# jinli99/iShapEditing

Hardware: AMD Instinct MI355X
Metric: end-to-end drag-edit wall-clock (s) per shape (lower is better)
Workload: dtype f16; 1 GPU; C3 chair drag-edit: 3 handle->target pairs, 40 guided iterations (UNet fwd + drag gradient + UNet input-grad bwd + DDPM update) + 256^3 occupancy decode; unet=421M params, 1x96x128x128 latent, fp16 torso, r1=12, scale=1200

## Files before the change

### ishapediting_amd/csrc/misc.hip

```cpp
#include "misc.h"

__global__ __launch_bounds__(256) void nchw_to_nhwc_kernel(const float* __restrict__ src, half_t* __restrict__ dst,
                                                           int C, int HW, int Cpad, int ytiles, uint4* __restrict__ zero, long long zero_n16) {
  __shared__ float tile[32][33];
  const int n = blockIdx.z;
  if ((int)blockIdx.y >= ytiles) {
    const long long nb = (long long)gridDim.x * (gridDim.y - ytiles) * gridDim.z;
    const long long b = blockIdx.x + (long long)gridDim.x * ((blockIdx.y - ytiles) + (long long)(gridDim.y - ytiles) * blockIdx.z);
    for (long long i = b * 256 + threadIdx.x; i < zero_n16; i += nb * 256) zero[i] = make_uint4(0u, 0u, 0u, 0u);
    return;
  }
  const int p0 = blockIdx.x * 32, c0 = blockIdx.y * 32;
  const int tx = threadIdx.x & 31, ty = threadIdx.x >> 5;
  for (int j = ty; j < 32; j += 8) {
    int c = c0 + j, p = p0 + tx;
    tile[j][tx] = (c < C && p < HW) ? src[((long long)n * C + c) * HW + p] : 0.f;
  }
  __syncthreads();
  for (int j = ty; j < 32; j += 8) {
    int p = p0 + j, c = c0 + tx;
    if (p < HW && c < Cpad) dst[((long long)n * HW + p) * Cpad + c] = (half_t)tile[tx][j];
  }
}
int nchw_f32_to_nhwc_f16(const float* src, half_t* dst, int N, int C, int HW, int Cpad, hipStream_t s, void* zero, size_t zero_bytes) {
// ... 43 lines not shown
  const int tx = threadIdx.x & 31, ty = threadIdx.x >> 5;
  for (int j = ty; j < 32; j += 8) {
    int c = c0 + j, p = p0 + tx;
    tile[j][tx] = (c < C && p < HW) ? (float)src[((long long)n * C + c) * HW + p] * mul : 0.f;
  }
  __syncthreads();
  for (int j = ty; j < 32; j += 8) {
    int p = p0 + j, c = c0 + tx;
    if (p < HW && c < ld) dst[((long long)n * HW + p) * ld + c] = (half_t)tile[tx][j];
  }
}
int nchw_to_nhwc_f16_scaled(const void* src, int src_f32, half_t* dst, int N, int C, int HW, int ld, float mul,
                            hipStream_t s) {
  dim3 g(ceil_div(HW, 32), ceil_div(ld, 32), N);
  if (src_f32) hipLaunchKernelGGL(nchw_any_to_nhwc_kernel<float>, g, dim3(256), 0, s, (const float*)src, dst, C, HW, ld, mul);
  else hipLaunchKernelGGL(nchw_any_to_nhwc_kernel<half_t>, g, dim3(256), 0, s, (const half_t*)src, dst, C, HW, ld, mul);
  ISHAP_CHECK_HIP(hipGetLastError());
  return 0;
}

__global__ void concat2_kernel(const half_t* __restrict__ a, const half_t* __restrict__ b, half_t* __restrict__ o,
                               long long M, int Ca, int Cb, const long long* __restrict__ sa,
                               const long long* __restrict__ sb, long long* __restrict__ so, int N) {
  if (so && blockIdx.x == 0) {
    const int Cc = Ca + Cb;
    for (int i = threadIdx.x; i < N * Cc * 2; i += blockDim.x) {
      const int k = i & 1, c = (i >> 1) % Cc, n = (i >> 1) / Cc;
      so[i] = c < Ca ? sa[(n * Ca + c) * 2 + k] : sb[(n * Cb + (c - Ca)) * 2 + k];
    }
  }
  const int CV = (Ca + Cb) >> 3, CVa = Ca >> 3;
  const long long total = M * CV;
  for (long long i = (long long)blockIdx.x * blockDim.x + threadIdx.x; i < total; i += (long long)gridDim.x * blockDim.x) {
    long long m = i / CV;
    int cv = (int)(i % CV);
    half8 v = cv < CVa ? *reinterpret_cast<const half8*>(a + m * Ca + cv * 8)
                       : *reinterpret_cast<const half8*>(b + m * Cb + (cv - CVa) * 8);
    *reinterpret_cast<half8*>(o + m * (Ca + Cb) + cv * 8) = v;
  }
}
int concat2(const half_t* a, const half_t* b, half_t* o, long long M, int Ca, int Cb, hipStream_t s, const long long* sa,
            const long long* sb, long long* so, int N) {
  long long total = M * ((Ca + Cb) / 8);
  int blocks = (int)std::min<long long>((total + 255) / 256, 4096);
  hipLaunchKernelGGL(concat2_kernel, dim3(blocks), dim3(256), 0, s, a, b, o, M, Ca, Cb, sa, sb, so, N);
  ISHAP_CHECK_HIP(hipGetLastError());
  return 0;
}

__global__ void add_kernel(const half_t* __restrict__ a, const half_t* __restrict__ b, half_t* __restrict__ o, long long nvec) {
  for (long long i = (long long)blockIdx.x * blockDim.x + threadIdx.x; i < nvec; i += (long long)gridDim.x * blockDim.x) {
    half8 x = reinterpret_cast<const half8*>(a)[i], y = reinterpret_cast<const half8*>(b)[i], r;
#pragma unroll
    for (int k = 0; k < 8; ++k) r[k] = (half_t)((float)x[k] + (float)y[k]);
    reinterpret_cast<half8*>(o)[i] = r;
  }
}
int add_f16(const half_t* a, const half_t* b, half_t* o, long long n, hipStream_t s) {
  long long nvec = n / 8;
  int blocks = (int)std::min<long long>((nvec + 255) / 256, 4096);
  hipLaunchKernelGGL(add_kernel, dim3(blocks), dim3(256), 0, s, a, b, o, nvec);
  ISHAP_CHECK_HIP(hipGetLastError());
  return 0;
}


__global__ void timestep_embedding_kernel(TsArg t, float* __restrict__ out, int dim) {
  const int n = blockIdx.x;
  const int half = dim / 2;
  for (int j = threadIdx.x; j < half; j += blockDim.x) {
    float f = expf(-logf(10000.f) * (float)j / (float)half);
    float a = t.t[n] * f;
    out[n * dim + j] = cosf(a);
    out[n * dim + half + j] = sinf(a);
  }
  if ((dim & 1) && threadIdx.x == 0) out[n * dim + dim - 1] = 0.f;
}
int timestep_embedding(const TsArg& t, float* out, int N, int dim, hipStream_t s) {
  hipLaunchKernelGGL(timestep_embedding_kernel, dim3(N), dim3(128), 0, s, t, out, dim);
  ISHAP_CHECK_HIP(hipGetLastError());
  return 0;
}

__global__ __launch_bounds__(256) void gemv_kernel(const float* __restrict__ W, const float* __restrict__ b,
                                                   const float* __restrict__ in, float* __restrict__ out, int rows, int K,
                                                   int N, int silu_in) {
  const int row = blockIdx.x * 4 + (threadIdx.x >> 6);
  const int lane = threadIdx.x & 63;
  if (row >= rows) return;
  const float* w = W + (long long)row * K;
  for (int n = 0; n < N; ++n) {
    float acc = 0.f;
    for (int k = lane * 4; k < K; k += 256) {
      f32x4 wv = *reinterpret_cast<const f32x4*>(w + k);
      f32x4 xv = *reinterpret_cast<const f32x4*>(in + (long long)n * K + k);
#pragma unroll
      for (int i = 0; i < 4; ++i) {
        float x = xv[i];
        if (silu_in) x = x / (1.f + __expf(-x));
        acc += wv[i] * x;
      }
    }
    for (int o = 32; o > 0; o >>= 1) acc += __shfl_xor(acc, o);
    if (lane == 0) out[(long long)n * rows + row] = acc + b[row];
  }
}
int gemv_f32(const float* W, const float* b, const float* in, float* out, int rows, int K, int N, int silu_in,
             hipStream_t s) {
  ISHAP_REQUIRE(K % 4 == 0, "gemv K % 4");
  hipLaunchKernelGGL(gemv_kernel, dim3(ceil_div(rows, 4)), dim3(256), 0, s, W, b, in, out, rows, K, N, silu_in);
  ISHAP_CHECK_HIP(hipGetLastError());
  return 0;
}

__global__ void pack_conv_kernel(const float* __restrict__ w, half_t* __restrict__ dst, int O, int I, int taps,
                                 int rows_pad, int cpad, int transpose_flip, int dst_ld, int col_off) {
  const long long total = (long long)rows_pad * taps * cpad;
  for (long long i = (long long)blockIdx.x * blockDim.x + threadIdx.x; i < total; i += (long long)gridDim.x * blockDim.x) {
    int c = (int)(i % cpad);
    int tap = (int)((i / cpad) % taps);
    int r = (int)(i / ((long long)cpad * taps));
    float v = 0.f;
    if (!transpose_flip) {
      if (r < O && c < I) v = w[((long long)r * I + c) * taps + tap];
    } else {
      if (r < I && c < O) v = w[((long long)c * I + r) * taps + (taps - 1 - tap)];
    }
    dst[(long long)r * dst_ld + col_off + tap * cpad + c] = (half_t)v;
  }
}
int pack_conv_weight(const float* w, half_t* dst, int O, int I, int taps, int rows_pad, int cpad, int transpose_flip,
                     hipStream_t s, int dst_ld, int col_off) {
  long long total = (long long)rows_pad * taps * cpad;
  int blocks = (int)std::min<long long>((total + 255) / 256, 8192);
  hipLaunchKernelGGL(pack_conv_kernel, dim3(blocks), dim3(256), 0, s, w, dst, O, I, taps, rows_pad, cpad, transpose_flip,
                     dst_ld ? dst_ld : taps * cpad, col_off);
  ISHAP_CHECK_HIP(hipGetLastError());
  return 0;
}

__global__ void pack_conv_split_kernel(const float* __restrict__ w, half_t* __restrict__ dst, int O, int I, int taps,
                                       int rows_pad) {
  const int cpad = 3 * I;
  const long long total = (long long)rows_pad * taps * cpad;
  for (long long i = (long long)blockIdx.x * blockDim.x + threadIdx.x; i < total; i += (long long)gridDim.x * blockDim.x) {
    int c3 = (int)(i % cpad);
    int tap = (int)((i / cpad) % taps);
    int r = (int)(i / ((long long)cpad * taps));
    int part = c3 / I, c = c3 % I;
    float v = 0.f;
    if (r < O) {
      float f = w[((long long)r * I + c) * taps + tap];
      half_t hi = (half_t)f;
      v = (part < 2) ? (float)hi : (f - (float)hi);
    }
    dst[i] = (half_t)v;
  }
}
int pack_conv_weight_split(const float* w, half_t* dst, int O, int I, int taps, int rows_pad, hipStream_t s) {
  long long total = (long long)rows_pad * taps * 3 * I;
  int blocks = (int)std::min<long long>((total + 255) / 256, 8192);
  hipLaunchKernelGGL(pack_conv_split_kernel, dim3(blocks), dim3(256), 0, s, w, dst, O, I, taps, rows_pad);
  ISHAP_CHECK_HIP(hipGetLastError());
  return 0;
}

__global__ void round_f16_kernel(const float* __restrict__ src, float* __restrict__ dst, long long n) {
  for (long long i = (long long)blockIdx.x * blockDim.x + threadIdx.x; i < n; i += (long long)gridDim.x * blockDim.x)
    dst[i] = (float)(half_t)src[i];
}
int round_through_f16(const float* src, float* dst, long long n, hipStream_t s) {
  int blocks = (int)std::min<long long>((n + 255) / 256, 4096);
  hipLaunchKernelGGL(round_f16_kernel, dim3(blocks), dim3(256), 0, s, src, dst, n);
  ISHAP_CHECK_HIP(hipGetLastError());
  return 0;
}

__global__ __launch_bounds__(256) void nhwc_to_nchw_scaled_kernel(const half_t* __restrict__ src, float* __restrict__ dst,
                                                                  int C, int HW, int ld, const float* __restrict__ mul_dev) {
  __shared__ float tile[32][33];
  const float mul = mul_dev ? *mul_dev : 1.f;
  const int n = blockIdx.z;
  const int p0 = blockIdx.x * 32, c0 = blockIdx.y * 32;
  const int tx = threadIdx.x & 31, ty = threadIdx.x >> 5;
  for (int j = ty; j < 32; j += 8) {
    int p = p0 + j, c = c0 + tx;
    tile[j][tx] = (c < C && p < HW) ? (float)src[((long long)n * HW + p) * ld + c] * mul : 0.f;
  }
  __syncthreads();
  for (int j = ty; j < 32; j += 8) {
    int c = c0 + j, p = p0 + tx;
    if (c < C && p < HW) dst[((long long)n * C + c) * HW + p] = tile[tx][j];
  }
}
// ... 8 lines not shown
```

### ishapediting_amd/csrc/unet.hip

```cpp
#include "unet.h"

#include <cstring>

#include "attention.h"
#include "decode.h"
#include "misc.h"
#include "norm.h"

static int round_up(int a, int b) { return (a + b - 1) / b * b; }

static void init_conv(ConvW& c, const std::string& path, int cin, int cout, int taps) {
  c.path = path; c.cin = cin; c.cout = cout; c.taps = taps;
  c.kpad = round_up(cin, 32);
  c.cout_pad = round_up(cout, 32);
}

int unet_build(ishap_unet* u) {
  const ishap_unet_config& cfg = u->cfg;
  const int mc = cfg.model_channels;
  u->ted = mc * 4;
  u->in_pad = cfg.in_channels >= 64 ? round_up(cfg.in_channels, 64) : round_up(cfg.in_channels, 32);
  auto has_att = [&](int ds) {
    for (int i = 0; i < cfg.n_att; ++i) if (cfg.attention_ds[i] == ds) return true;
    return false;
  };
  auto heads_of = [&](int ch) { return ch / cfg.num_head_channels; };
  u->res.reserve(256);
  u->attn.reserve(64);
  int film = 0;
  auto add_res = [&](const std::string& path, int cin, int cout, bool up, bool down) {
    ResL r;
    r.path = path; r.cin = cin; r.cout = cout; r.up = up; r.down = down;
    r.n1.C = cin; r.n2.C = cout;
    init_conv(r.c1, path + ".in_layers.2", cin, cout, 9);
    init_conv(r.c2, path + ".out_layers.3", cout, cout, 9);
    r.has_skip = cin != cout;
    if (r.has_skip) init_conv(r.skip, path + ".skip_connection", cin, cout, 1);
    r.emb_off = film;
    film += 2 * cout;
    u->res.push_back(r);
    return (int)u->res.size() - 1;
  };
  auto add_attn = [&](const std::string& path, int ch) {
    AttnL a;
    a.path = path; a.C = ch; a.heads = heads_of(ch);
    a.n.C = ch;
    init_conv(a.qkv, path + ".qkv", ch, 3 * ch, 1);
    init_conv(a.proj, path + ".proj_out", ch, ch, 1);
    u->attn.push_back(a);
    return (int)u->attn.size() - 1;
  };

  int ch = cfg.channel_mult[0] * mc;
  int res = cfg.image_size;
  init_conv(u->stem, "input_blocks.0.0", cfg.in_channels, ch, 9);
  u->stem.kpad = u->in_pad;
  {
    BlockL b;
    b.name = "input_blocks.0";
    b.layers.push_back({0, 0});
    b.cin = cfg.in_channels; b.cout = ch; b.res_in = b.res_out = res;
    u->in_blocks.push_back(b);
  }
  std::vector<int> chans{ch};
  int ds = 1;
  for (int level = 0; level < cfg.n_mult; ++level) {
    for (int k = 0; k < cfg.num_res_blocks; ++k) {
      BlockL b;
      b.name = "input_blocks." + std::to_string(u->in_blocks.size());
      int cout = cfg.channel_mult[level] * mc;
      b.layers.push_back({1, add_res(b.name + ".0", ch, cout, false, false)});
      b.cin = ch; ch = cout; b.cout = ch; b.res_in = b.res_out = res;
      if (has_att(ds)) b.layers.push_back({2, add_attn(b.name + ".1", ch)});
      u->in_blocks.push_back(b);
      chans.push_back(ch);
    }
    if (level != cfg.n_mult - 1) {
      BlockL b;
      b.name = "input_blocks." + std::to_string(u->in_blocks.size());
      b.layers.push_back({1, add_res(b.name + ".0", ch, ch, false, true)});
      b.cin = b.cout = ch; b.res_in = res; b.res_out = res / 2;
      u->in_blocks.push_back(b);
      chans.push_back(ch);
      ds *= 2;
// ... 600 lines not shown
  u->marks_on = ishap_switch("ISHAP_BWD_MARKS", 0) != 0;
  u->device = device;
  int r = unet_build(u);
  if (r) { delete u; return r; }
  u->arena.dry = true;
  std::vector<float> ts(cfg->max_batch, 0.f);
  for (int nb = 1; nb <= cfg->max_batch && !r; ++nb) {
    r = unet_forward_impl(u, nullptr, ts.data(), nb, (int)u->out_blocks.size() - 1, nullptr, nullptr, 1, 0, true);
    if (!r) r = unet_backward_impl(u, nullptr, (const void*)0x1000, 0, nullptr, nullptr, 0, true);
  }
  if (r) { delete u; return r; }
  u->arena.dry = false;
  u->arena.cap = align_up(u->arena.high + (1 << 20), 1 << 20);
  ISHAP_CHECK_HIP(hipMalloc((void**)&u->arena.base, u->arena.cap));
  if (u->ws_floats) ISHAP_CHECK_HIP(hipMalloc((void**)&u->ws, u->ws_floats * sizeof(float)));
  ISHAP_CHECK_HIP(hipMalloc((void**)&u->gn_partial, std::max<size_t>(u->gn_partial_floats, 64) * sizeof(float)));
  u->stat_cap = (u->stat_high + 1023) / 1024 * 1024;
  ISHAP_CHECK_HIP(hipMalloc((void**)&u->stat_base, std::max<size_t>(u->stat_cap, 1024) * sizeof(long long)));
  if (u->attn_D_floats) ISHAP_CHECK_HIP(hipMalloc((void**)&u->attn_D, u->attn_D_floats * sizeof(float)));
  u->have_saved = false;
  *out = u;
  return 0;
}

void ishap_unet_destroy(ishap_unet* u) {
  if (!u) return;
  auto fr = [](void* p) { if (p) (void)hipFree(p); };
  auto frc = [&](ConvW& c) { fr(c.w); fr(c.wT); fr(c.bias); if (c.cat && c.cat_off == 0) fr(c.cat); };
  frc(u->stem); frc(u->head);
  fr(u->head_norm.gamma); fr(u->head_norm.beta);
  for (auto& r : u->res) {
    frc(r.c1); frc(r.c2); if (r.has_skip) frc(r.skip);
    fr(r.n1.gamma); fr(r.n1.beta); fr(r.n2.gamma); fr(r.n2.beta);
  }
  for (auto& a : u->attn) { frc(a.qkv); frc(a.proj); fr(a.n.gamma); fr(a.n.beta); }
  fr(u->te_w0); fr(u->te_b0); fr(u->te_w2); fr(u->te_b2); fr(u->emb_w); fr(u->emb_b);
  fr(u->d_temb); fr(u->d_e1); fr(u->d_emb); fr(u->d_film);
  fr(u->film_cache); fr(u->pc_temb); fr(u->pc_e1); fr(u->pc_emb);
  fr(u->ws_side); fr(u->gn_partial_side);
  fr(u->snap.arena); fr(u->snap.stat); fr(u->snap.film);
  if (u->side) (void)hipStreamDestroy(u->side);
  if (u->ev_fork) (void)hipEventDestroy(u->ev_fork);
  if (u->ev_tail) (void)hipEventDestroy(u->ev_tail);
  if (u->ev_mid) (void)hipEventDestroy(u->ev_mid);
  for (hipEvent_t ev : u->marks) (void)hipEventDestroy(ev);
  if (u->mark_tail_begin) (void)hipEventDestroy(u->mark_tail_begin);
  if (u->mark_tail_end) (void)hipEventDestroy(u->mark_tail_end);
  fr(u->arena.base); fr(u->ws); fr(u->gn_partial); fr(u->attn_D); fr(u->stat_base);
  delete u;
}

int ishap_unet_num_params(const ishap_unet* u) { return u ? (int)u->params.size() : 0; }

int ishap_unet_param_info(const ishap_unet* u, int index, char* name, int name_cap, int* ndim, long long* shape) {
  ISHAP_REQUIRE(u && index >= 0 && index < (int)u->params.size(), "param index");
  const ParamSlot& p = u->params[index];
  if (name && name_cap > 0) {
    std::strncpy(name, p.name.c_str(), name_cap - 1);
    name[name_cap - 1] = 0;
  }
  if (ndim) *ndim = p.ndim;
  if (shape) for (int i = 0; i < 4; ++i) shape[i] = p.shape[i];
  return 0;
}

int ishap_unet_load_param(ishap_unet* u, const char* name, const float* data, long long numel, void* stream) {
  ISHAP_REQUIRE(u && name && data, "null argument");
  auto it = u->param_index.find(name);
  ISHAP_REQUIRE(it != u->param_index.end(), std::string("unexpected key in state_dict: ") + name);
  ParamSlot& p = u->params[it->second];
  ISHAP_REQUIRE(p.numel() == numel, std::string("size mismatch for ") + name);
  ISHAP_CHECK_HIP(hipSetDevice(u->device));
  ISHAP_TRY(load_param(u, p, data, (hipStream_t)stream));
  if (!p.loaded) { p.loaded = true; u->n_loaded++; }
  u->film_cache_ts.clear();
  u->snap.valid = false;
  return 0;
}

int ishap_unet_prepare_timesteps(ishap_unet* u, const float* ts, int n, void* stream) {
  ISHAP_REQUIRE(u && (ts || n == 0) && n >= 0 && n <= 4096, "prepare_timesteps arguments");
  ISHAP_CHECK_HIP(hipSetDevice(u->device));
  hipStream_t s = (hipStream_t)stream;
  u->film_cache_ts.clear();
  if (u->film_cur != u->d_film) { u->have_saved = false; u->film_cur = u->d_film; u->film_cur_ld = u->film_rows; }
  if (n == 0) return 0;
  ISHAP_REQUIRE(u->n_loaded == (int)u->params.size(), "prepare_timesteps before all parameters are loaded");
  const int mc = u->cfg.model_channels;
  if ((size_t)n > u->film_cache_rows) {
    if (u->film_cache) ISHAP_CHECK_HIP(hipFree(u->film_cache));
    u->film_cache = nullptr;
    u->film_cache_rows = 0;
    ISHAP_CHECK_HIP(hipMalloc((void**)&u->film_cache, (size_t)n * u->film_rows * sizeof(float)));
    u->film_cache_rows = (size_t)n;
  }
  if (!u->pc_temb) {
    ISHAP_CHECK_HIP(hipMalloc((void**)&u->pc_temb, (size_t)16 * mc * sizeof(float)));
    ISHAP_CHECK_HIP(hipMalloc((void**)&u->pc_e1, (size_t)16 * u->ted * sizeof(float)));
    ISHAP_CHECK_HIP(hipMalloc((void**)&u->pc_emb, (size_t)16 * u->ted * sizeof(float)));
  }
  for (int c0 = 0; c0 < n; c0 += 16) {
    const int m = std::min(16, n - c0);
    TsArg ta;
    for (int i = 0; i < 16; ++i) ta.t[i] = i < m ? ts[c0 + i] : 0.f;
    ISHAP_TRY(timestep_embedding(ta, u->pc_temb, m, mc, s));
    ISHAP_TRY(gemv_f32(u->te_w0, u->te_b0, u->pc_temb, u->pc_e1, u->ted, mc, m, 0, s));
    ISHAP_TRY(gemv_f32(u->te_w2, u->te_b2, u->pc_e1, u->pc_emb, u->ted, u->ted, m, 1, s));
    ISHAP_TRY(gemv_f32(u->emb_w, u->emb_b, u->pc_emb, u->film_cache + (size_t)c0 * u->film_rows, u->film_rows, u->ted, m, 1, s));
  }
  u->film_cache_ts.assign(ts, ts + n);
  return 0;
}

int ishap_unet_params_loaded(const ishap_unet* u) { return u ? u->n_loaded : 0; }

int ishap_unet_join_tail(ishap_unet* u, void* stream) {
  ISHAP_REQUIRE(u, "null argument");
  ISHAP_CHECK_HIP(hipSetDevice(u->device));
  return unet_join_tail(u, (hipStream_t)stream);
}

int ishap_unet_run_tail(ishap_unet* u) {
  ISHAP_REQUIRE(u, "null argument");
  ISHAP_CHECK_HIP(hipSetDevice(u->device));
  return unet_run_tail(u);
}

int ishap_unet_forward(ishap_unet* u, const float* x, const float* timesteps, int N, int feat_layer, float* out,
                       void* inter_feat, int keep_for_backward, void* stream) {
  ISHAP_REQUIRE(u && x && timesteps && out, "null argument");
  ISHAP_REQUIRE(u->n_loaded == (int)u->params.size(), "missing keys: not every state_dict tensor has been loaded");
  ISHAP_TRY(ishap_check_status());
  ISHAP_CHECK_HIP(hipSetDevice(u->device));
  return unet_forward_impl(u, x, timesteps, N, feat_layer, out, inter_feat, keep_for_backward, (hipStream_t)stream, false);
}

int ishap_unet_tap_shape(const ishap_unet* u, int feat_layer, int* channels, int* size) {
  ISHAP_REQUIRE(u && feat_layer >= 0 && feat_layer < (int)u->out_blocks.size(), "feat_layer out of range");
  if (channels) *channels = u->out_blocks[feat_layer].cout;
  if (size) *size = u->out_blocks[feat_layer].res_out;
  return 0;
}

const void* ishap_unet_tap_ptr(const ishap_unet* u) { return u ? u->tap.p : nullptr; }

long long ishap_unet_workspace_bytes(const ishap_unet* u) {
  if (!u) return 0;
  return (long long)(u->arena.cap + u->ws_floats * sizeof(float) + u->gn_partial_floats * sizeof(float) +
                     u->stat_cap * sizeof(long long) + u->attn_D_floats * sizeof(float) + u->snap.bytes());
}

int ishap_unet_block_output(const ishap_unet* u, int group, int index, int* channels, int* size, void* dst_nchw_f16,
                            void* stream) {
  ISHAP_REQUIRE(u && group >= 0 && group <= 2, "group: 0 input_blocks, 1 middle_block, 2 output_blocks");
  const BlockL* b = nullptr;
  if (group == 0) { ISHAP_REQUIRE(index >= 0 && index < (int)u->in_blocks.size(), "input block index"); b = &u->in_blocks[index]; }
  else if (group == 1) b = &u->mid;
  else { ISHAP_REQUIRE(index >= 0 && index < (int)u->out_blocks.size(), "output block index"); b = &u->out_blocks[index]; }
  if (channels) *channels = b->cout;
  if (size) *size = b->res_out;
  if (!dst_nchw_f16) return 0;
  ISHAP_REQUIRE(u->have_saved && b->out.p, "block outputs stay resident only after a forward with keep_for_backward=1");
  ISHAP_REQUIRE(!(u->restored_partial && group == 2 && index > u->last_feat), "the restored snapshot holds the network up to the tap only");
  ISHAP_TRY(ishap_check_status());
  ISHAP_CHECK_HIP(hipSetDevice(u->device));
  ISHAP_TRY(unet_join_tail(const_cast<ishap_unet*>(u), (hipStream_t)stream));
// ... 125 lines not shown
```

### ishapediting_amd/drag_utils.py

```python
from __future__ import annotations

import argparse
import collections
import copy
import ctypes as C
import os
from argparse import Namespace
from typing import List, Optional

import numpy as np
import torch as th

from . import _lib
from .script_util import args_to_dict, create_model_and_diffusion, model_and_diffusion_defaults
from .triplane_decoder import MultiTriplane, decode_planes_grid, decode_volume, prepare_planes
from . import mesh as mesh_backend
from .volume import clean_volume


def get_args(argv=None):
    parser = argparse.ArgumentParser(description="Generate a set of triplane and their corresponding meshes")
    parser.add_argument("--resolution", type=str, default=128, required=False)
    parser.add_argument("--num_steps", type=int, default=200, required=False)
    parser.add_argument("--shape_resolution", type=int, default=256, required=False)
# ... 319 lines not shown
        if t.dtype != th.float16 or tuple(t.shape[-2:]) != (self.W * self.W, self.ld):
            raise ValueError(f"taps are fp16 [..., {self.W * self.W}, {self.ld}], got {t.dtype} {tuple(t.shape)}")
        t = t.to(self.device).contiguous()
        if t.dim() == 2:
            t = t[None]
        if t.dim() != 3 or t.shape[0] not in lead:
            raise ValueError(f"tap batch of {tuple(t.shape)} for {self.E} edits")
        return t

    def track_batch(self, edit_taps, orig_taps, sources, offsets=None, want_volume=False) -> List[Track]:
        self.setup(sources)
        edit, orig = self._tap(edit_taps, (self.E,)), self._tap(orig_taps, (1, self.E))
        H = self.handles
        if offsets is None:
            K_in = th.zeros((H, 3), dtype=th.int32, device=self.device)
        else:
            K_in = th.cat([th.as_tensor(np.asarray(o.detach().cpu() if th.is_tensor(o) else o)).to(th.int32).reshape(-1, 3)
                           for o in offsets]).to(self.device).contiguous()
            if K_in.shape[0] != H:
                raise ValueError(f"{K_in.shape[0]} offsets for {H} handles")
        K_out = th.empty_like(K_in)
        dist, dist0 = th.empty(H, dtype=th.float32, device=self.device), th.empty(H, dtype=th.float32, device=self.device)
        vol = th.empty((H, self.side ** 3), dtype=th.float32, device=self.device) if want_volume else None
        self.run_ptr(edit.data_ptr(), orig.data_ptr(), 0 if orig.shape[0] == 1 else orig[0].numel(), K_in, K_out, dist, dist0, vol)
        pos = self.positions(K_out)
        cut = lambda t, e: None if t is None else t[self.offsets[e]:self.offsets[e + 1]]
        return [Track(cut(K_out, e), cut(pos, e), cut(dist, e), cut(dist0, e), cut(vol, e)) for e in range(self.E)]

    def track(self, edit_tap, orig_tap, sources, offsets=None, want_volume=False) -> Track:
        return self.track_batch(edit_tap, orig_tap, [sources], None if offsets is None else [offsets], want_volume)[0]


class _LoopTrack:

    def __init__(self, tracker: HandleTracker, sources, steps_total: int, every: int):
        self.tracker, self.every = tracker.setup(sources), every
        rows = (steps_total + every - 1) // every
        H, dev = tracker.handles, tracker.device
        self.table = th.zeros((rows + 1, H, 3), dtype=th.int32, device=dev)
        self.dist = th.zeros((rows, H), dtype=th.float32, device=dev)
        self.dist0 = th.zeros((rows, H), dtype=th.float32, device=dev)
        self.steps: List[int] = []
        self._ptrs = (self.table.data_ptr(), self.dist.data_ptr(), self.dist0.data_ptr(), H)

    def step(self, n: int, edit_ptr: int, orig_ptr: int, orig_stride: int):
        if n % self.every:
            return
        r = len(self.steps)
        table, dist, dist0, H = self._ptrs
        self.tracker.run_raw(edit_ptr, orig_ptr, orig_stride, table + 12 * H * r, table + 12 * H * (r + 1), dist + 4 * H * r,
                             dist0 + 4 * H * r)
        self.steps.append(n)

    def results(self) -> List[dict]:
        t, r = self.tracker, len(self.steps)
        offs = self.table[1:r + 1].clone()
        pos = t.positions(offs)
        out = []
        for e in range(t.E):
            a, b = t.offsets[e], t.offsets[e + 1]
            out.append({"steps": list(self.steps), "offsets": offs[:, a:b], "positions": pos[:, a:b],
                        "dist": self.dist[:r, a:b].clone(), "dist0": self.dist0[:r, a:b].clone(), "radius": t.R, "patch": t.rp})
        return out


def synthesize_latent(model, diffusion, args=None, t1=None, t2=0, inter_latent_idx=None, inter_feat_idx=None, img=None,
                      calc_grad=False, **kwargs):
    if args is None:
        args = get_args()
    shape = (args.batch_size, 96, args.image_size, args.image_size)
    if img is None:
        img = th.randn(shape, device=next(model.parameters()).device)
        if calc_grad:
            img.requires_grad_(True)
    assert img.shape == shape
    if t1 is None:
        t1 = args.num_steps
    elif t1 == 0:
        return {"img": img[:args.num_samples], "inter_latent": [], "inter_feat": [], "pred_xstart": [], "model_output": None}
    sample_fun = diffusion.ddim_sample if getattr(args, "use_ddim", False) else diffusion.p_sample_guidance
    if calc_grad and getattr(args, "use_ddim", False):
        raise NotImplementedError("synthesize_latent(calc_grad=True) with use_ddim: the DDIM sampler has no autograd bridge")
    inter_latent, inter_feat, predict_x0, model_output, variance, noise = [], [], [], None, [], []
    with (th.enable_grad() if calc_grad else th.no_grad()):
        for i in range(t1 - 1, t2 - 1, -1):
            out = sample_fun(model, img, i, **kwargs)
            img = out["sample"]
            if inter_feat_idx is not None and i in inter_feat_idx:
                inter_feat.append(out["inter_feat"])
                if calc_grad:
                    noise.append(out["noise"].cpu())
                    variance.append(out["variance"].cpu())
            if inter_latent_idx is not None and i in inter_latent_idx:
                inter_latent.append(img)
                predict_x0.append(out["pred_xstart"])
            model_output = out["model_output"]
    return {"img": img[:args.num_samples], "inter_latent": inter_latent, "inter_feat": inter_feat,
            "pred_xstart": predict_x0, "model_output": model_output, "variance": variance, "noise": noise}


def load_triplane_stats(stats=None, stats_dir=None):
    if stats is not None:
        means, stds = stats
    else:
        files = [os.path.join(stats_dir, f) for f in ("means.npy", "stds.npy")] if stats_dir else []
        if not files or not all(os.path.exists(f) for f in files):
            raise FileNotFoundError(
                "train_triplane_opt needs the triplane statistics: pass stats=(means, stds) or set args.stats_dir to a "
                f"directory holding means.npy and stds.npy (stats_dir={stats_dir!r})")
        means, stds = (np.load(f) for f in files)
    means, stds = (np.asarray(v, dtype=np.float32).reshape(-1) for v in (means, stds))
    if means.size != 96 or stds.size != 96:
        raise ValueError(f"triplane statistics must hold 96 values each, not {means.size} and {stds.size}")
    return means, stds


class DragStuff:

    args = get_args()
    overlap_tail = None
    _w = None
    _shape_gen = 0
    _first_step = None

    @property
    def w(self):
        return self._w

    @w.setter
    def w(self, value):
        self._w = value
        self._shape_changed()

    def _shape_changed(self):
        self._shape_gen = self._shape_gen + 1
        self._first_step = None

    def _first_step_key(self, overlap):
        w = self._w
        return (self._shape_gen, id(self.model), id(w), getattr(w, "_version", None), tuple(w.shape), self.args.feat_layer,
                self.args.w_time, tuple(getattr(self.diffusion, "timestep_map", ())), bool(overlap))

    def __init__(self, device=None, args=None, max_edits=1):
        if args is not None:
            self.args = args
        if int(max_edits) < 1:
            raise ValueError(f"max_edits must be >= 1, not {max_edits}")
        self.max_edits = int(max_edits)
        self.device = th.device("cuda", th.cuda.current_device()) if device is None else th.device(device)
        self.model, self.diffusion = create_model_and_diffusion(
            **args_to_dict(self.args, model_and_diffusion_defaults().keys()), device=self.device, max_batch=self.max_edits)
        self.model.eval()
        self.decoder = MultiTriplane(1, input_dim=3, output_dim=1, device=self.device)
        self.decoder.eval()
        self.range = 1.
        self.middle = 0.
        self.latent_code = None
        self.w0 = None
        self.w = None
        self.r1 = 12
        self.offset1 = make_offsets(self.r1, self.device)
        self.voxel_size = 2. / self.args.shape_resolution
        self.train_flag = True
        self.targets = None
        self.sources = None
        self.mesh = None
        self.mesh0 = None
        self.volume = None
        self.clean = None
        self.refine = None
        self.noise = []
        self.variance = []
        self.variance_noise = []
        self.feature_guidance: List[th.Tensor] = []
        self.last_losses: List[float] = []
        self.last_track = None
        self._dk: Optional[DragKernels] = None
        self.step_noise = None
        self.w_batch = None
        self.w0_batch = None
        self.feature_guidance_batch: List[th.Tensor] = []
        self.meshes0 = []
        self.meshes = []
        self.volumes = []

    def set_offset1(self, r1):
        self.r1 = int(r1)
        self.offset1 = make_offsets(r1, self.device)

    def update_model_params(self, main_path):
        for files in os.listdir(main_path):
            if files.startswith("ddpm"):
                ddpm_path = os.path.join(main_path, files)
                for sub_file in os.listdir(ddpm_path):
                    if sub_file.startswith("ema"):
                        self.args.model_path = os.path.join(ddpm_path, sub_file)
                        break
            elif files.endswith(".pt"):
                self.args.decoder_ckpt = os.path.join(main_path, files)
        stat_path = os.path.join(main_path, "statistics")
        self.args.stats_dir = os.path.join(stat_path, os.listdir(stat_path)[0])
        self.args.save_dir = os.path.join("samples", main_path[9:] + "_samples")
        os.makedirs(self.args.save_dir, exist_ok=True)
        self.load_weights(th.load(self.args.model_path, map_location="cpu"),
                          th.load(self.args.decoder_ckpt, map_location="cpu"),
                          np.load(f"{self.args.stats_dir}/lower_bound.npy") if self.args.explicit_normalization else None,
                          np.load(f"{self.args.stats_dir}/upper_bound.npy") if self.args.explicit_normalization else None)

    def load_weights(self, unet_sd, decoder_sd, lower_bound=None, upper_bound=None):
        self._shape_changed()
        self.model.load_state_dict(unet_sd, strict=True)
        if self.args.use_fp16:
            self.model.convert_to_fp16()
        self.model.eval()
        if lower_bound is not None:
            mn = np.asarray(lower_bound).astype(np.float32).reshape(1, -1, 1, 1)
            mx = np.asarray(upper_bound).astype(np.float32).reshape(1, -1, 1, 1)
            self.range = (th.tensor(mx - mn) / 2).to(self.device)
            self.middle = th.tensor((mn + mx) / 2).to(self.device)
        else:
            self.range, self.middle = 1., 0.
        self.decoder.net.load_state_dict(decoder_sd)
        self.decoder.eval()

    def _noise(self, i, like):
        return None if self.step_noise is None else self.step_noise(i).to(like.device)

    def _denoise(self, img, t, each=None, **kwargs):
        for i in range(t - 1, -1, -1):
            img = self.diffusion.p_sample_guidance(self.model, img, i, feat_layer=self.args.feat_layer,
                                                   clip_denoised=self.args.clip_denoised, want_inter_feat=False,
                                                   noise=self._noise(i, img), want_noise=False, **kwargs)["sample"]
            if each is not None:
                each(i, img)
        return img

    def update_latent_params(self, img=None, **kwargs):
        if img is not None:
            if th.is_tensor(img):
                img = img.type(th.float32).to(self.device)
            elif type(img) is np.ndarray:
                img = th.tensor(img, dtype=th.float32, device=self.device)
            else:
                raise NotImplementedError("Unknown data type!")
        else:
            img = th.randn((1, 96, self.args.image_size, self.args.image_size), dtype=th.float32, device=self.device)
        self.latent_code = img.clone().detach()
        self._shape_changed()
        self.w_batch, self.w0_batch, self.feature_guidance_batch = None, None, []

        def record(i, img):
            if i == self.args.w_time:
                self.w = img.clone().detach()
                self.w0 = self.w.clone().detach()
            if i < self.args.w_time:
                self.feature_guidance.append(self.model.copy_tap(self.args.feat_layer)[0])

        img = self._denoise(img, self.args.num_steps, each=record, **kwargs)
        assert len(self.feature_guidance) == self.args.w_time
        self.mesh0 = self.get_mesh(tri_feat=img)
        self.mesh = copy.deepcopy(self.mesh0)
        return img

    def get_mesh(self, tri_feat=None, img=None, t=0):
        if tri_feat is None:
            img = img if img is not None else th.randn((1, 96, self.args.image_size, self.args.image_size)).to(self.device)
            tri_feat = self._denoise(img, t)
        self.tri_feat = tri_feat
        refine = None
        if self.refine is None:
            self.volume = decode_volume(self.decoder, tri_feat.to(self.device), self.range, self.middle,
                                        self.args.shape_resolution)
        else:
            planes = prepare_planes(tri_feat.to(self.device), self.range, self.middle)
            self.volume = decode_planes_grid(self.decoder, planes, self.args.shape_resolution)
            refine = dict(self.refine, decoder=self.decoder, planes=planes)
        if self.clean is not None:
            self.volume = clean_volume(self.volume, **self.clean)
        return mesh_backend.volume_to_mesh(self.volume, self.args.shape_resolution, smooth_iterations=10, refine=refine)

    def _guided_loop(self, img, dk, guidance, stride, scales, guided_scale, reuse_first=False, trk=None):
        w_time = self.args.w_time
        overlap = _OVERLAP_TAIL if self.overlap_tail is None else self.overlap_tail
        reuse_first = reuse_first and _FIRST_STEP_REUSE and hasattr(self.model, "snapshot_restore")
        stop_time = 0
        self.train_flag = True
        losses = th.zeros((w_time, len(scales)), dtype=th.float32, device=self.device)
        self.diffusion.prepare(self.model, range(w_time))
        self.last_losses = []
        for i in range(w_time - 1, -1, -1):
            if not self.train_flag:
                stop_time = i + 1
                break
            origin = guidance[w_time - 1 - i]
            slot = losses[i]
            got = {}

            def loss_and_backward():
                cot, scale2 = dk.loss_cotangent_ptr(self.model.tap_ptr(), origin.data_ptr(), orig_stride=stride, loss_out=slot)
                if trk is not None:
                    trk.step(w_time - 1 - i, self.model.tap_ptr(), origin.data_ptr(), stride)
                got["grad"] = self.model.backward_input(cot, scale2)
                return got["grad"]

            first = {}
            if reuse_first and i == w_time - 1:
                key, kept = self._first_step_key(overlap), self._first_step
                if kept is not None and kept["key"] == key and self.model.has_snapshot() and self.model.snapshot_restore():
                    first["model_output"] = kept["out"]
                else:
                    def keep_first(mo, key=key):
# ... 124 lines not shown
    def training_batch(self, sources, targets, scale=600, cof=0.2, keep=None, free=None, keep_weight=4.0, free_weight=0.0,
                       region_dilate=0, weights=None, track=None):
        topts = track_options(track)
        if len(sources) != len(targets):
            raise ValueError(f"{len(sources)} source sets but {len(targets)} target sets: one of each per edit")
        K = len(sources)
        self._check_edits(K)
        scales = per_edit(scale, K, "scale")
        cofs = per_edit(cof, K, "cof")
        ch, width = self.model.tap_shape(self.args.feat_layer)
        keeps, frees, maps = (per_edit_region(v, K, n) for v, n in ((keep, "keep"), (free, "free"), (weights, "weights")))
        kws, fws = per_edit(keep_weight, K, "keep_weight"), per_edit(free_weight, K, "free_weight")
        dils = per_edit_any(region_dilate, K, "region_dilate")
        wmaps = [self._region_weights(width, cofs[k], keeps[k], frees[k], kws[k], fws[k], dils[k], maps[k], f"cof[{k}]")
                 for k in range(K)]
        if self.w_batch is not None:
            if self.w_batch.shape[0] != K:
                raise ValueError(f"{K} edits for the {self.w_batch.shape[0]} shapes of update_latent_params_batch")
            img = self.w_batch.clone().detach()
            guidance, stride = self.feature_guidance_batch, width * width * ch
        else:
            if self.w is None:
                raise RuntimeError("training_batch needs update_latent_params (variants of one shape) or update_latent_params_batch first")
            img = self.w.expand(K, *self.w.shape[1:]).contiguous()
            guidance, stride = self.feature_guidance, 0
        dk = BatchDragKernels(self.device, K, W=width, ld=ch, chmap=feat_channel_map(ch), r=self.r1, voxel=self.voxel_size,
                              loss_type=self.args.loss_type)
        dk.setup(sources, targets, cofs, **({} if all(w is None for w in wmaps) else {"weights": wmaps}))
        self._dk_batch = dk
        trk = self._loop_track(topts, width, ch, sources)
        scales_dev = th.tensor(scales, dtype=th.float32, device=self.device)
        img, stop_time = yield from self._guided_loop(img, dk, guidance, stride, scales, scales_dev,
                                                      **({} if trk is None else {"trk": trk}))
        if trk is not None:
            self.last_track = trk.results()
            self._track_ends = [(dk.sources[a:b], dk.targets[a:b]) for a, b in zip(dk.offsets[:-1], dk.offsets[1:])]
        self.get_meshes(img=img, t=stop_time)

    def _cloud_samples(self, cloud, center, generator=None):
        pts, nrm = mesh_backend.load_cloud(cloud)
        return mesh_backend.sample_cloud_occupancy(pts, nrm, self.args.points_size, self.args.points_uniform_ratio, center=center,
                                                   generator=generator, device=self.device)

    def train_triplane(self, mesh=None, mesh_path=None, center_mesh=True, tri_feat_path=None, path="./",
                       points=None, occupancies=None, occupancy="parity", cloud=None):
        mesh_backend._check_choice("occupancy", occupancy, mesh_backend.OCCUPANCY_METHODS)
        if tri_feat_path is not None:
            img = th.tensor(np.load(tri_feat_path), device=self.device)
            if img.dim() == 3:
                img = img.unsqueeze(0)
            self.mesh = self.get_mesh(img)
            self.mesh0 = copy.deepcopy(self.mesh)
            self.latent_inversion(tri_feat=img)
            return
        if points is None and cloud is not None:
            points, occupancies = self._cloud_samples(cloud, center_mesh)
        if points is None:
            points, occupancies = mesh_backend.sample_occupancy(mesh, mesh_path, center_mesh, self.args.points_size,
                                                                self.args.points_uniform_ratio, device=self.device,
                                                                occupancy=occupancy)
            if points is None:
                return
        points = th.as_tensor(np.asarray(points), dtype=th.float32).to(self.device)
        occupancies = th.as_tensor(np.asarray(occupancies), dtype=th.float32).reshape(-1).to(self.device)
        img = self.reconstruct(points, occupancies)
        np.save(os.path.join(path, "tri_feat.npy"), img.cpu().numpy())
        self.clear_params()
        self.mesh = self.get_mesh(tri_feat=img)
        self.mesh0 = copy.deepcopy(self.mesh)
        mesh_backend.write_mesh(os.path.join(path, "mesh_recon.obj"), self.mesh0)
        self.latent_inversion(tri_feat=img)

    def reconstruct(self, points, occupancies, scale=600, batch_size=40000, img=None, batch_fn=None, steps=None):
        L = _lib.lib()
        d = self.diffusion
        if img is None:
            img = th.randn((1, 96, self.args.image_size, self.args.image_size), dtype=th.float32, device=self.device)
        img = img.to(self.device).float().contiguous()
        rng_t = self.range if th.is_tensor(self.range) else None
        S = self.args.image_size
        bits = th.zeros(1, dtype=th.int32, device=self.device)
        scale2 = th.ones(2, dtype=th.float32, device=self.device)
        self.last_losses = []
        for i in (steps if steps is not None else range(self.args.num_steps - 1, -1, -1)):
            outs = d.p_sample_guidance(self.model, img, i, keep_for_backward=True, noise=self._noise(i, img), want_noise=False)
            if batch_fn is not None:
                coord, gt = batch_fn(i)
            else:
                idx = th.randperm(points.shape[0], device=self.device)[:batch_size]
                coord, gt = points[idx], occupancies[idx]
            from .triplane_decoder import prepare_planes
            planes = prepare_planes(outs["pred_xstart"], self.range, self.middle)
            loss, dplanes, _ = self.decoder.points_loss_grad(planes, coord, gt)
            g_direct = th.empty_like(img)
            cot = th.empty((1, 192, S, S), dtype=th.float32, device=self.device)
            sr = float(np.float32(d.sqrt_recip_alphas_cumprod[i]))
            srm1 = float(np.float32(d.sqrt_recipm1_alphas_cumprod[i]))
            new = th.empty_like(img)
            cot16 = th.empty((1, 192, S, S), dtype=th.float16, device=self.device)
            with th.cuda.device(self.device):
                s = _lib.stream_ptr(self.device)
                _lib.check(L.ishap_x0_grad_to_cotangent(dplanes.data_ptr(), _lib.ptr(rng_t.reshape(-1).contiguous()) if rng_t is not None else None,
                                                        img.data_ptr(), outs["model_output"].data_ptr(), sr, srm1,
                                                        int(self.args.clip_denoised), S, g_direct.data_ptr(), cot.data_ptr(), s))
                _lib.check(L.ishap_grad_to_scaled_f16(cot.data_ptr(), cot16.data_ptr(), bits.data_ptr(), scale2.data_ptr(),
                                                      cot.numel(), s))
            dx = self.model.backward_from_output(cot16, scale2)
            grads1 = th.empty_like(dx)
            with th.cuda.device(self.device):
                _lib.check(L.ishap_axpby(dx.data_ptr(), g_direct.data_ptr(), 1.0, 1.0, dx.numel(), grads1.data_ptr(),
                                         _lib.stream_ptr(self.device)))
                _lib.check(L.ishap_guided_update(outs["sample"].data_ptr(), outs["variance"].data_ptr(), grads1.data_ptr(),
                                                 float(scale), None, img.numel(), new.data_ptr(), _lib.stream_ptr(self.device)))
            img = new
            self.last_losses.append(loss)
        return img

    def train_triplane_opt(self, mesh=None, mesh_path=None, center_mesh=True, path="./", points=None, occupancies=None,
                           stats=None, epochs=20, batch_size=40000, lr=1e-3, seed=None, batch_fn=None, occupancy="parity",
                           cloud=None):
        from .triplane_decoder import fit_triplanes, planes_to_latent
        mesh_backend._check_choice("occupancy", occupancy, mesh_backend.OCCUPANCY_METHODS)
        means, stds = load_triplane_stats(stats, self.args.stats_dir)
        sample_gen = None if seed is None else th.Generator().manual_seed(int(seed))
        if points is None and cloud is not None:
            points, occupancies = self._cloud_samples(cloud, center_mesh, sample_gen)
        if points is None:
            points, occupancies = mesh_backend.sample_occupancy(
                mesh, mesh_path, center_mesh, self.args.points_size, self.args.points_uniform_ratio, device=self.device,
                generator=sample_gen, occupancy=occupancy)
            if points is None:
                return None
        points = th.as_tensor(np.asarray(points) if not th.is_tensor(points) else points, dtype=th.float32).to(self.device)
        occupancies = th.as_tensor(np.asarray(occupancies) if not th.is_tensor(occupancies) else occupancies,
                                   dtype=th.float32).reshape(-1).to(self.device)
        S = self.args.image_size
        gen = th.Generator(device=self.device)
        if seed is not None:
            gen.manual_seed(int(seed))
        else:
            gen.seed()
        mean = th.as_tensor(np.asarray(means), dtype=th.float32).reshape(1, 96, 1, 1).to(self.device)
        std = th.as_tensor(np.asarray(stds), dtype=th.float32).reshape(1, 96, 1, 1).to(self.device)
        init = th.randn((1, 96, S, S), generator=gen, device=self.device) * std + mean
        planes, self.last_losses = fit_triplanes(self.decoder, points, occupancies, init, epochs=epochs,
                                                 batch_size=batch_size, lr=lr, generator=gen, batch_fn=batch_fn)
        fitted = planes_to_latent(planes)
        self.decoder.embeddings = [fitted[:, 32 * i:32 * (i + 1)].clone() for i in range(3)]
        latent = (fitted - self.middle) / self.range
        np.save(os.path.join(path, "tri_feat_opt.npy"), latent.cpu().numpy())
        mesh_backend.write_mesh(os.path.join(path, "mesh_opt.obj"), self.get_mesh(latent))
        return latent

    def latent_inversion(self, tri_feat, fwd_noise=None):
        self._shape_changed()
        outs = self.diffusion.ddpm_inversion(self.model, tri_feat, self.args.w_time, fwd_noise=fwd_noise,
                                             clip_denoised=self.args.clip_denoised, feat_layer=self.args.feat_layer,
                                             want_inter_feat=False, tap_sink=self._tap_sink_reset())
        self.w = outs["latent"].clone().detach()
        self.w0 = self.w.clone().detach()
        self.feature_guidance = list(self._sink)
        self.mesh = self.get_mesh(tri_feat=outs["sample"])
        self.mesh0 = copy.deepcopy(self.mesh)
        self.variance = [v.clone().detach() for v in outs["variance"]]
        self.variance_noise = [v.clone().detach() for v in outs["variance_noise"]]

    def _tap_sink_reset(self):
# ... 21 lines not shown
```

Measured before the change: 0.1573 s/shape.

## Batch FiLM timestep GEMV across rows/batches and skip redundant timestep preparation

Rewrites the fp32 GEMV used for timestep/FiLM embeddings. It now stages SiLU-applied inputs in LDS once per block, processes two rows per wavefront for up to 16 inputs at a time, and double-buffers the weight loads, so weights are read once for many inputs rather than once per input. prepare_timesteps returns early when every requested timestep is already in the FiLM cache. The Python sampling loops now call diffusion.prepare up front so all per-step FiLM vectors are computed in batch. Limits K to 4096 and adds more LDS use, and the early-return check relies on cache bookkeeping staying correct.

```diff
diff --git a/ishapediting_amd/csrc/misc.hip b/ishapediting_amd/csrc/misc.hip
--- a/ishapediting_amd/csrc/misc.hip
+++ b/ishapediting_amd/csrc/misc.hip
@@ -149,34 +149,96 @@
   return 0;
 }
 
-__global__ __launch_bounds__(256) void gemv_kernel(const float* __restrict__ W, const float* __restrict__ b,
-                                                   const float* __restrict__ in, float* __restrict__ out, int rows, int K,
-                                                   int N, int silu_in) {
-  const int row = blockIdx.x * 4 + (threadIdx.x >> 6);
+constexpr int GEMV_LDS_FLOATS = 16384;
+template <int J, int NB>
+__global__ __launch_bounds__(256) void gemv_rows_kernel(const float* __restrict__ W, const float* __restrict__ b,
+                                                        const float* __restrict__ in, float* __restrict__ out, int rows, int K,
+                                                        int N, int silu_in) {
+  extern __shared__ __attribute__((aligned(16))) float gemv_xs[];
+  for (int i = threadIdx.x * 4; i < NB * K; i += 1024) {
+    f32x4 v = {0.f, 0.f, 0.f, 0.f};
+    if (i < N * K) v = *reinterpret_cast<const f32x4*>(in + i);
+    if (silu_in) {
+#pragma unroll
+      for (int c = 0; c < 4; ++c) {
+        float x = v[c];
+        v[c] = x / (1.f + __expf(-x));
+      }
+    }
+    *reinterpret_cast<f32x4*>(gemv_xs + i) = v;
+  }
+  __syncthreads();
   const int lane = threadIdx.x & 63;
-  if (row >= rows) return;
-  const float* w = W + (long long)row * K;
-  for (int n = 0; n < N; ++n) {
-    float acc = 0.f;
-    for (int k = lane * 4; k < K; k += 256) {
-      f32x4 wv = *reinterpret_cast<const f32x4*>(w + k);
-      f32x4 xv = *reinterpret_cast<const f32x4*>(in + (long long)n * K + k);
-#pragma unroll
-      for (int i = 0; i < 4; ++i) {
-        float x = xv[i];
-        if (silu_in) x = x / (1.f + __expf(-x));
-        acc += wv[i] * x;
+  const int npairs = (rows + 1) / 2, stride = gridDim.x * 4;
+  int p = blockIdx.x * 4 + (threadIdx.x >> 6);
+  if (p >= npairs) return;
+  auto load = [&](f32x4 (&w)[2][J], int pair) {
+#pragma unroll
+    for (int r = 0; r < 2; ++r) {
+      const float* wp = W + (long long)min(pair * 2 + r, rows - 1) * K;
+#pragma unroll
+      for (int j = 0; j < J; ++j) {
+        const int k = lane * 4 + 256 * j;
+        w[r][j] = k < K ? *reinterpret_cast<const f32x4*>(wp + k) : f32x4{0.f, 0.f, 0.f, 0.f};
       }
     }
-    for (int o = 32; o > 0; o >>= 1) acc += __shfl_xor(acc, o);
-    if (lane == 0) out[(long long)n * rows + row] = acc + b[row];
+  };
+  f32x4 wc[2][J], wn[2][J];
+  load(wc, p);
+  for (; p < npairs; p += stride) {
+    if (p + stride < npairs) load(wn, p + stride);
+    float acc[2][NB];
+#pragma unroll
+    for (int n = 0; n < NB; ++n) acc[0][n] = acc[1][n] = 0.f;
+#pragma unroll
+    for (int j = 0; j < J; ++j) {
+      const int k = lane * 4 + 256 * j;
+      if (k < K) {
+#pragma unroll
+        for (int n = 0; n < NB; ++n) {
+          const f32x4 xv = *reinterpret_cast<const f32x4*>(gemv_xs + n * K + k);
+#pragma unroll
+          for (int r = 0; r < 2; ++r)
+#pragma unroll
+            for (int i = 0; i < 4; ++i) acc[r][n] = __builtin_fmaf(wc[r][j][i], xv[i], acc[r][n]);
+        }
+      }
+    }
+#pragma unroll
+    for (int r = 0; r < 2; ++r) {
+      const int row = p * 2 + r;
+      float mine = 0.f;
+#pragma unroll
+      for (int n = 0; n < NB; ++n) {
+        float a = acc[r][n];
+#pragma unroll
+        for (int o = 32; o > 0; o >>= 1) a += __shfl_xor(a, o);
+        if (lane == n) mine = a;
+      }
+      if (row < rows && lane < N) out[(long long)lane * rows + row] = mine + b[row];
+    }
+#pragma unroll
+    for (int r = 0; r < 2; ++r)
+#pragma unroll
+      for (int j = 0; j < J; ++j) wc[r][j] = wn[r][j];
   }
 }
 int gemv_f32(const float* W, const float* b, const float* in, float* out, int rows, int K, int N, int silu_in,
              hipStream_t s) {
-  ISHAP_REQUIRE(K % 4 == 0, "gemv K % 4");
-  hipLaunchKernelGGL(gemv_kernel, dim3(ceil_div(rows, 4)), dim3(256), 0, s, W, b, in, out, rows, K, N, silu_in);
-  ISHAP_CHECK_HIP(hipGetLastError());
+  ISHAP_REQUIRE(K % 4 == 0 && K > 0 && K <= 4096, "gemv: K % 4, K <= 4096");
+  ISHAP_REQUIRE(rows > 0 && N >= 0, "gemv: rows, N");
+  const int nb = K <= 1024 ? 16 : 4;
+  const int grid = std::min(ceil_div(ceil_div(rows, 2), 4), 512);
+  for (int n0 = 0; n0 < N; n0 += nb) {
+    const int m = std::min(nb, N - n0);
+    const size_t lds = (size_t)nb * K * sizeof(float);
+    const float* x = in + (long long)n0 * K;
+    float* o = out + (long long)n0 * rows;
+    if (K <= 256) hipLaunchKernelGGL((gemv_rows_kernel<1, 16>), dim3(grid), dim3(256), lds, s, W, b, x, o, rows, K, m, silu_in);
+    else if (K <= 1024) hipLaunchKernelGGL((gemv_rows_kernel<4, 16>), dim3(grid), dim3(256), lds, s, W, b, x, o, rows, K, m, silu_in);
+    else hipLaunchKernelGGL((gemv_rows_kernel<16, 4>), dim3(grid), dim3(256), lds, s, W, b, x, o, rows, K, m, silu_in);
+    ISHAP_CHECK_HIP(hipGetLastError());
+  }
   return 0;
 }
 
diff --git a/ishapediting_amd/csrc/unet.hip b/ishapediting_amd/csrc/unet.hip
--- a/ishapediting_amd/csrc/unet.hip
+++ b/ishapediting_amd/csrc/unet.hip
@@ -1,5 +1,6 @@
 #include "unet.h"
 
+#include <algorithm>
 #include <cstring>
 
 #include "attention.h"
@@ -766,6 +767,12 @@
   ISHAP_REQUIRE(u && (ts || n == 0) && n >= 0 && n <= 4096, "prepare_timesteps arguments");
   ISHAP_CHECK_HIP(hipSetDevice(u->device));
   hipStream_t s = (hipStream_t)stream;
+  if (n > 0 && !u->film_cache_ts.empty()) {
+    const std::vector<float>& have = u->film_cache_ts;
+    bool current = true;
+    for (int i = 0; i < n && current; ++i) current = std::find(have.begin(), have.end(), ts[i]) != have.end();
+    if (current) return 0;
+  }
   u->film_cache_ts.clear();
   if (u->film_cur != u->d_film) { u->have_saved = false; u->film_cur = u->d_film; u->film_cur_ld = u->film_rows; }
   if (n == 0) return 0;
diff --git a/ishapediting_amd/drag_utils.py b/ishapediting_amd/drag_utils.py
--- a/ishapediting_amd/drag_utils.py
+++ b/ishapediting_amd/drag_utils.py
@@ -425,6 +425,7 @@
     if calc_grad and getattr(args, "use_ddim", False):
         raise NotImplementedError("synthesize_latent(calc_grad=True) with use_ddim: the DDIM sampler has no autograd bridge")
     inter_latent, inter_feat, predict_x0, model_output, variance, noise = [], [], [], None, [], []
+    diffusion.prepare(model, range(t2, t1))
     with (th.enable_grad() if calc_grad else th.no_grad()):
         for i in range(t1 - 1, t2 - 1, -1):
             out = sample_fun(model, img, i, **kwargs)
@@ -570,6 +571,7 @@
         return None if self.step_noise is None else self.step_noise(i).to(like.device)
 
     def _denoise(self, img, t, each=None, **kwargs):
+        self.diffusion.prepare(self.model, range(t))
         for i in range(t - 1, -1, -1):
             img = self.diffusion.p_sample_guidance(self.model, img, i, feat_layer=self.args.feat_layer,
                                                    clip_denoised=self.args.clip_denoised, want_inter_feat=False,
@@ -860,7 +862,9 @@
         bits = th.zeros(1, dtype=th.int32, device=self.device)
         scale2 = th.ones(2, dtype=th.float32, device=self.device)
         self.last_losses = []
-        for i in (steps if steps is not None else range(self.args.num_steps - 1, -1, -1)):
+        steps = list(steps) if steps is not None else list(range(self.args.num_steps - 1, -1, -1))
+        d.prepare(self.model, steps)
+        for i in steps:
             outs = d.p_sample_guidance(self.model, img, i, keep_for_backward=True, noise=self._noise(i, img), want_noise=False)
             if batch_fn is not None:
                 coord, gt = batch_fn(i)
```

Result: no change. 0.1577 s/shape (+0.3%).
